# jdm365/Compression_Algorithms

Hardware: AMD Instinct MI355X
Metric: encode GB/s on enwik9 at 1/2/4/8 MI355X; ratio vs ref; round-trip bit-exact (higher is better)
Workload: dtype u8; 1 GPU; deflate (LZ77 W=32 KiB len<=31 + per-block dynamic Huffman over the 286-symbol alphabet, mode H), independent 64 KiB blocks; 1000000000 enwik-shaped bytes in the job, 1000000000 on rank 0; input_seed=12345, mode=H, input_bytes_job=1000000000, input_bytes_rank0=1000000000, compressed_bytes_job=516875560, compressed_bytes_rank0=516875560, gather_to_rank0=False, parallelism=blocks sharded over 1 GPU(s), weak scaling

## Files before the change

compression_algorithms_amd/csrc/lz2.h:

```cpp
#pragma once
#include "lz_common.h"

#define LZ2_NG_BITS   14
#define LZ2_NG        (1u << LZ2_NG_BITS)
#ifndef LZ2_CAP
#define LZ2_CAP       4096u
#endif
#ifndef LZ2_CAP_S
#define LZ2_CAP_S     2048u
#endif
#ifndef LZ2_THREADS
#define LZ2_THREADS   512
#endif
#define LZ2_NWAVES    (LZ2_THREADS / 64)
#ifndef LZ2_PARTBITS
#define LZ2_PARTBITS  7
#endif
#define LZ2_MAXPARTS  (1u << LZ2_PARTBITS)
static_assert(LZ2_CAP % LZ2_THREADS == 0 && LZ2_CAP_S % LZ2_THREADS == 0 && LZ2_CAP_S <= LZ2_CAP, "entries per thread must be whole");
static_assert(2u * (LZ_MAX_BLOCK / LZ2_CAP_S + 1u + 16u) + 2u <= LZ2_MAXPARTS, "a block could need more parts than the partition can number");
#define LZ2_GRID_PARTS 40u
static_assert(LZ2_GRID_PARTS * LZ2_CAP_S >= 5u * LZ_MAX_BLOCK / 4u, "the grid must cover a full block of text with room to spare");
#ifndef LZ2_BIG
#define LZ2_BIG       8u
#endif
#define LZ2_WAVE      128u
#define LZ2_MAXBIG    (LZ2_CAP / LZ2_BIG)
#define LZ2_BIG_STRIDE (2u * LZ_MAX_BLOCK)
#define LZ2_ALIGN8(x)  (((x) + 7u) & ~7u)
#define LZ2_DESC_SMALL (LZ_MAX_BLOCK / LZ2_BIG + 32u)
#define LZ2_NCLASS    8u
#define LZ2_BIG_SMALL 1024u
__host__ __device__ __forceinline__ uint32_t lz2_class_of(uint32_t cnt, uint32_t wave_min)
{
    const bool three = (wave_min >> 16) != 0u;
    wave_min &= 0xFFFFu;
    if (cnt >= wave_min) return cnt > LZ2_BIG_SMALL ? 6u : cnt >= 512u ? 4u : (three && cnt < 256u) ? 3u : 5u;
    return cnt < 16 ? 7u : cnt < 32 ? 0u : cnt < 64 ? 1u : cnt < 128 ? 2u : cnt < 256 ? 3u : 4u;
}

struct Lz2BlockMeta {
    uint32_t n, nparts, base, fallback;
    uint32_t nbig, nbig_entries;
    uint32_t pad[2];
    uint32_t part_start[LZ2_MAXPARTS];
    uint32_t part_count[LZ2_MAXPARTS];
    uint32_t part_lo[LZ2_MAXPARTS];
};

struct Lz2BigDesc {
    uint32_t block;
    uint32_t start;
    uint32_t count;
    uint32_t anom;
    uint32_t limit;
    uint32_t pad[3];
};

struct Lz2Scratch {
    uint8_t      *partmap;
    uint16_t     *plist;
    uint16_t     *cand;
    Lz2BlockMeta *meta;
    uint32_t     *fallback_count, *fallback_list;
    uint32_t     *work_count;
    uint32_t      work_slots;
    uint64_t     *work;
    uint16_t     *bigpos, *bigrs, *bigpid, *bigcand;
    Lz2BigDesc   *desc[LZ2_NCLASS];
    uint32_t     *big_count;
    uint4        *lane_list;
    uint32_t     *lane_hist;
    uint64_t     *dbg;
    uint32_t      wave_min;
    uint32_t      stop_phase;
};
```

compression_algorithms_amd/csrc/lz2_find.hip:

```cpp
#include "lz_common.h"
#include "lz2.h"
#include "lz_dom.h"
#include "lz_replay.h"
#include "internal.h"
#include <stdlib.h>

#define RS_HEAD 0x8000u
#define RS_MASK 0x7FFFu

__device__ __forceinline__ bool bm2_test(const uint32_t *bm, uint32_t b) { return (bm[b >> 5] >> (b & 31u)) & 1u; }

__device__ void replay_small(const uint16_t *pos, uint16_t *rs, const uint16_t *pid, uint16_t *occ, uint32_t *bm,
                             uint32_t s, uint32_t e, uint32_t W, uint32_t anom, uint32_t limit, uint16_t *cand_i)
{
    uint32_t ev = s;
    bool anom_pending = anom != ~0u;
    const bool plain = (anom == ~0u) && (limit == ~0u);
    if (plain && (uint32_t)pos[e - 1] <= (uint32_t)pos[s] + W) {
        for (uint32_t i = s; i < e; ++i) { const uint32_t id = pid[i]; cand_i[i] = (id != pos[i]) ? (uint16_t)id : (uint16_t)LZ_NONE16; }
        return;
    }
    for (uint32_t i = s; i < e; ++i) {
        const uint32_t p = pos[i], rsv = rs[i], r = rsv & RS_MASK, id = pid[i];
        while (ev < i && (uint32_t)pos[ev] + W < p) {
// ... 546 lines not shown
        uint16_t *bp = sc.bigpos + (size_t)lb * LZ2_BIG_STRIDE + dst;
        uint16_t *br = sc.bigrs + (size_t)lb * LZ2_BIG_STRIDE + dst;
        uint16_t *bi = sc.bigpid + (size_t)lb * LZ2_BIG_STRIDE + dst;
        for (uint32_t i = s + (tid & 63); i < e; i += 64) {
            cand_i[i] = e_pos[i];
            bp[i - s] = e_pos[i];
            br[i - s] = (uint16_t)((e_rs[i] & RS_MASK) - s);
            bi[i - s] = e_pid[i];
        }
        uint16_t *bc = sc.bigcand + (size_t)lb * LZ2_BIG_STRIDE + dst;
        for (uint32_t k = (e - s) + (tid & 63); k < LZ2_ALIGN8(e - s); k += 64) { bp[k] = 0; bc[k] = 0; }
    }
    uint16_t *cand_j = s_pid;
    __syncthreads();
    for (uint32_t i = tid; i < m; i += LZ2_THREADS) cand_j[s_j1[i]] = cand_i[i];
    __syncthreads();
    uint16_t *cout = sc.cand + (size_t)lb * LZ_MAX_BLOCK + pstart;
    for (uint32_t j = tid; j < m; j += LZ2_THREADS) cout[j] = cand_j[j];
    LZ2_TICK(6);
    if (LZ2_DBG && tid == 0) atomicAdd((unsigned long long *)&LZ2_DBG[15], 1ull);
}


template <bool DESC>
__device__ __forceinline__ void lz2_find_listed(const uint8_t *__restrict__ in, uint64_t n_total, const LzP &P, const Lz2Scratch &sc, uint64_t block0)
{
    const uint32_t listed = *sc.work_count, nwork = listed < gridDim.x ? listed : gridDim.x;
    const uint32_t cpx = (nwork + 7u) >> 3, item_idx = (blockIdx.x & 7u) * cpx + (blockIdx.x >> 3);
    if ((blockIdx.x >> 3) >= cpx || item_idx >= nwork) return;
    lz2_find_part<LZ2_CAP_S, DESC>(in, n_total, P, sc, block0, sc.work[item_idx]);
}
__global__ __launch_bounds__(LZ2_THREADS, 8)
void k_lz2_find(const uint8_t *__restrict__ in, uint64_t n_total, LzP P, Lz2Scratch sc, uint64_t block0)
{
    lz2_find_listed<false>(in, n_total, P, sc, block0);
}
__global__ __launch_bounds__(LZ2_THREADS, 8)
void k_lz2_find_desc(const uint8_t *__restrict__ in, uint64_t n_total, LzP P, Lz2Scratch sc, uint64_t block0)
{
    lz2_find_listed<true>(in, n_total, P, sc, block0);
}

template <bool DESC>
__global__ __launch_bounds__(LZ2_THREADS)
void k_lz2_find_wide(const uint8_t *__restrict__ in, uint64_t n_total, LzP P, Lz2Scratch sc, uint64_t block0, uint32_t covered)
{
    const uint32_t nwide = sc.work_count[1], listed = sc.work_count[0], rest = listed > covered ? listed - covered : 0u;
    for (uint32_t k = blockIdx.x; k < nwide + rest; k += gridDim.x) {
        lz2_find_part<LZ2_CAP, DESC>(in, n_total, P, sc, block0, k < nwide ? sc.work[sc.work_slots - 1u - k] : sc.work[covered + (k - nwide)]);
        __syncthreads();
    }
}

template <int LDS_ENTRIES, int NW>
__global__ __launch_bounds__(64)
void k_lz2_big(LzP P, Lz2Scratch sc, int large)
{
    __shared__ uint32_t s_occ[LDS_ENTRIES];
    __shared__ uint16_t s_slot[LDS_ENTRIES];
    const uint32_t lane = threadIdx.x;
    const uint32_t nhi = large == 1 ? sc.big_count[6] : (large == 2 || large == 4) ? 0u : sc.big_count[4],
                   ncl = nhi + ((large == 0 || large == 2) ? sc.big_count[5] : large == 4 ? sc.big_count[3] : 0u);
    const uint32_t W = 1u << P.wbits;
    for (uint32_t ci = blockIdx.x; ci < ncl; ci += gridDim.x) {
        const Lz2BigDesc *dp = large == 1 ? &sc.desc[6][ci] : large == 4 ? &sc.desc[3][ci] : (ci < nhi ? &sc.desc[4][ci] : &sc.desc[5][ci - nhi]);
        const uint32_t d_block = dp->block, d_start = dp->start, n = dp->count;
        if (n & 0x80000000u) continue;
        const uint32_t d_anom = dp->anom, d_limit = dp->limit;
        const uint16_t *bp = sc.bigpos + (size_t)d_block * LZ2_BIG_STRIDE + d_start;
        const uint16_t *br = sc.bigrs + (size_t)d_block * LZ2_BIG_STRIDE + d_start;
        const uint16_t *bi = sc.bigpid + (size_t)d_block * LZ2_BIG_STRIDE + d_start;
        uint16_t *bc = sc.bigcand + (size_t)d_block * LZ2_BIG_STRIDE + d_start;
        const bool plain = d_anom == ~0u && d_limit == ~0u;
        if constexpr (NW > 1) {
            if (n <= 2048u) {
                if (plain) big_replay<LDS_ENTRIES, 1, true>(s_occ, s_slot, lane, W, n, d_anom, d_limit, bp, br, bi, bc);
                else big_replay<LDS_ENTRIES, 1, false>(s_occ, s_slot, lane, W, n, d_anom, d_limit, bp, br, bi, bc);
                continue;
            }
            if (n <= 4096u) {
                if (plain) big_replay<LDS_ENTRIES, 2, true>(s_occ, s_slot, lane, W, n, d_anom, d_limit, bp, br, bi, bc);
                else big_replay<LDS_ENTRIES, 2, false>(s_occ, s_slot, lane, W, n, d_anom, d_limit, bp, br, bi, bc);
                continue;
            }
        }
        if (plain) big_replay<LDS_ENTRIES, NW, true>(s_occ, s_slot, lane, W, n, d_anom, d_limit, bp, br, bi, bc);
        else big_replay<LDS_ENTRIES, NW, false>(s_occ, s_slot, lane, W, n, d_anom, d_limit, bp, br, bi, bc);
    }
}

#define LZ2_DOM_DONE 0x80000000u
__global__ __launch_bounds__(256)
void k_lz2_dom(LzP P, Lz2Scratch sc)
{
    constexpr uint32_t RING = LZ2_CAP;
    static_assert((RING & (RING - 1u)) == 0, "the ring is indexed with a mask");
    __shared__ uint32_t s_occ[LZ2_CAP / 32 + 72 + 264];
    __shared__ uint16_t s_ring[RING];
    __shared__ uint16_t s_fid[DOM_FCAP], s_fpos[DOM_FCAP], s_fslot[DOM_FCAP];
    __shared__ uint32_t s_votes[3], s_result, s_next;
    const uint32_t tid = threadIdx.x;
    const uint32_t W = 1u << P.wbits;
    const uint32_t count = sc.big_count[6];
    uint32_t *cursor = sc.big_count + 8;
    struct Src {
        const uint16_t *bp, *br, *bi; uint16_t *bc;
        __device__ __forceinline__ uint64_t ent(uint32_t i) const { return ((uint64_t)bp[i] << 16) | ((uint64_t)br[i] << 32) | ((uint64_t)bi[i] << 48); }
        __device__ __forceinline__ void put(uint32_t i, uint32_t, uint32_t res) const { bc[i] = (uint16_t)res; }
    };
    for (;;) {
        __syncthreads();
        if (tid == 0) s_next = atomicAdd(cursor, 1u);
        __syncthreads();
        const uint32_t ci = s_next;
        if (ci >= count) break;
        Lz2BigDesc *dp = &sc.desc[6][ci];
        const uint32_t m = dp->count;
        if (dp->anom != ~0u || dp->limit != ~0u || m > LZ2_CAP) continue;
        const size_t at = (size_t)dp->block * LZ2_BIG_STRIDE + dp->start;
        Src src{sc.bigpos + at, sc.bigrs + at, sc.bigpid + at, sc.bigcand + at};
        for (uint32_t i = tid; i < m; i += 256) src.bc[i] = (uint16_t)LZ_NONE16;
        if (tid == 0) { s_votes[0] = s_votes[1] = s_votes[2] = 0; s_result = 0; }
        __syncthreads();
        const bool done = dom_cluster(src, m, W, (W < RING ? W : RING) - 1u, s_occ, s_ring, s_fid, s_fpos, s_fslot, s_votes, s_result, nullptr);
        if (done && tid == 0) dp->count = m | LZ2_DOM_DONE;
    }
}

#define ROW_BPERM(src_lane, v) ((uint32_t)__builtin_amdgcn_ds_bpermute((int)((src_lane) << 2), (int)(v)))

template <int RL>
__device__ __forceinline__ uint32_t row_first_zero(uint32_t v, uint32_t from, uint32_t l, uint32_t rb)
{
    constexpr uint32_t RMASK = RL == 32 ? 0xFFFFFFFFu : ((1u << (RL & 31)) - 1u);
    const uint32_t rw = from >> 5, lowmask = (1u << (from & 31u)) - 1u;
    if (l < rw) v = 0xFFFFFFFFu; else if (l == rw) v |= lowmask;
    const uint64_t mk = __ballot(v != 0xFFFFFFFFu);
    const uint32_t my = (uint32_t)(mk >> rb) & RMASK;
    const uint32_t ln = my ? (uint32_t)__builtin_ctz(my) : 0u;
    const uint32_t mv = ROW_BPERM(rb + ln, v);
    const uint32_t fz = (mv != 0xFFFFFFFFu) ? (uint32_t)__builtin_ctz(~mv) : 0u;
    return my ? ((ln << 5) + fz) : ~0u;
}

template <int RL>
__global__ __launch_bounds__(64)
void k_lz2_rows(LzP P, Lz2Scratch sc, int cls_a, int cls_b, int cursor_slot)
{
    static_assert(RL == 8 || RL == 16 || RL == 32, "rows of 8, 16 or 32 lanes");
    constexpr int NR = 64 / RL, CAPE = 32 * RL;
    constexpr uint32_t RMASK = RL == 32 ? 0xFFFFFFFFu : ((1u << (RL & 31)) - 1u);
    __shared__ uint32_t s_occ[NR][CAPE];
    __shared__ uint32_t s_ent[NR][CAPE];
    __shared__ uint32_t s_bm[NR][RL];
    const uint32_t lane = threadIdx.x, g = lane / (uint32_t)RL, l = lane & (uint32_t)(RL - 1), rb = lane & ~(uint32_t)(RL - 1);
    const uint32_t W = 1u << P.wbits;
    const uint32_t count_a = sc.big_count[cls_a], count = count_a + sc.big_count[cls_b];
    uint32_t *cursor = sc.big_count + cursor_slot;
    Lz2BigDesc *const descs_a = sc.desc[cls_a], *const descs_b = sc.desc[cls_b];
    auto desc_of = [&](uint32_t ticket) -> Lz2BigDesc * { return ticket < count_a ? descs_a + ticket : descs_b + (ticket - count_a); };
    uint32_t *occ = s_occ[g], *ent = s_ent[g], *bmw = s_bm[g];

    bool active = false, exhausted = false;
    uint32_t n = 0, i0 = 0, ev = 0;
    size_t at = 0;
    uint32_t cur_a = 0, cur_b = 0, out_acc = LZ_NONE16;
    uint32_t pf_stage = 0, pf_ci = 0, pf_count = 0;
    size_t pf_at = 0;
    uint32_t r_np = 0, r_ni = 0, r_nr = 0, r_fp = 0, r_fi = 0, r_fr = 0, tk = 0;
    uint4 r_d4 = make_uint4(0, 0, 0, 0); uint32_t r_d1 = 0;
    uint32_t vzero;
    asm volatile("v_mov_b32 %0, 0" : "=v"(vzero));

    for (;;) {
        const bool flush = active && i0 + l < n;
        uint16_t *const flush_to = sc.bigcand + at + i0 + l;
        if (active) {
            i0 += (uint32_t)RL;
            if (i0 >= n) active = false;
            else { cur_a = r_np | (r_ni << 16); cur_b = r_nr; }
        }
        bool take = false, want_cursor = false;
        uint32_t done_ci = 0, done_n = 0;
        if (!active && pf_stage == 3u) {
            take = true;
            n = pf_count; at = pf_at;
            cur_a = r_fp | (r_fi << 16); cur_b = r_fr; i0 = 0; ev = 0; active = true; pf_stage = 0;
            bmw[l] = 0;
            done_ci = pf_ci; done_n = n;
        }
        if (pf_stage == 1u) {
            pf_ci = ROW_BPERM(rb, tk);
            if (pf_ci >= count) { exhausted = true; pf_stage = 0; } else pf_stage = 2;
        } else if (pf_stage == 2u) {
            if (r_d4.w != ~0u || r_d1 != ~0u || r_d4.z > (uint32_t)CAPE || r_d4.z < 2u * RL) pf_stage = 0;
            else { pf_count = r_d4.z; pf_at = (size_t)r_d4.x * LZ2_BIG_STRIDE + r_d4.y; pf_stage = 3; }
        }
        if (pf_stage == 0u && !exhausted) { want_cursor = true; pf_stage = 1; }
        {
            const uint32_t k = i0 + (uint32_t)RL + l;
            const size_t na = (active && k < n) ? at + k : 0;
            r_np = sc.bigpos[na]; r_ni = sc.bigpid[na]; r_nr = sc.bigrs[na];
            const size_t fa = (pf_stage == 3u) ? pf_at + l : 0;
            r_fp = sc.bigpos[fa]; r_fi = sc.bigpid[fa]; r_fr = sc.bigrs[fa];
            const uint32_t *dp = reinterpret_cast<const uint32_t *>(pf_stage == 2u ? desc_of(pf_ci) : descs_a);
            r_d4 = *reinterpret_cast<const uint4 *>(dp); r_d1 = dp[4];
        }
        if (flush) *flush_to = (uint16_t)out_acc;
        if (take && l == 0) desc_of(done_ci)->count = done_n | LZ2_DOM_DONE;
        if (want_cursor && l == 0) tk = atomicAdd(cursor + vzero, 1u);
        if (__ballot(active || pf_stage != 0u) == 0ull) break;
        if (__ballot(active) == 0ull) continue;
        uint32_t a = ROW_BPERM(rb, cur_a), r = ROW_BPERM(rb, cur_b);
        uint32_t e = ent[(active && ev + l < i0) ? ev + l : 0u];
        for (uint32_t t = 0; t < (uint32_t)RL; ++t) {
            const uint32_t i = i0 + t;
            const bool on = active && i < n;
            const uint32_t p = a & 0xFFFFu, id = a >> 16;
            for (;;) {
                const bool ret = on && ev + l < i && (e >> 16) + W < p;
                const uint64_t mk = __ballot(ret);
                if (ret) atomicAnd(&bmw[(e & 0xFFFFu) >> 5], ~(1u << (e & 31u)));
                const uint32_t cnt = (uint32_t)__popc((uint32_t)(mk >> rb) & RMASK);
                ev += cnt;
                if (__ballot(cnt == (uint32_t)RL) == 0ull) break;
                e = ent[(on && ev + l < i) ? ev + l : 0u];
            }
            const uint32_t wr = bmw[r >> 5], h = occ[r], v = bmw[l];
            const uint32_t tn = (t + 1u) & (uint32_t)(RL - 1);
            const uint32_t na = ROW_BPERM(rb + tn, cur_a), nr = ROW_BPERM(rb + tn, cur_b);
            const bool bit = (wr >> (r & 31u)) & 1u, same = (h & 0xFFFFu) == id;
            const bool seek = on && id != p;
            uint32_t res = (seek && ev == 0u) ? id : (seek && bit && same) ? (h >> 16) : (uint32_t)LZ_NONE16;
            bool walk = seek && ev != 0u && bit && !same;
            if (__ballot(walk) != 0ull) {
                uint32_t e_end = row_first_zero<RL>(v, r + 1u, l, rb);
                if (e_end > (uint32_t)CAPE) e_end = (uint32_t)CAPE;
                uint32_t b0 = r + 1u;
                while (__ballot(walk && b0 < e_end) != 0ull) {
                    const uint32_t bb = b0 + l;
                    const bool in = walk && bb < e_end;
                    const uint32_t o = occ[in ? bb : 0u];
                    const uint64_t mk = __ballot(in && (o & 0xFFFFu) == id);
                    const uint32_t my = (uint32_t)(mk >> rb) & RMASK;
                    const uint32_t src = ROW_BPERM(rb + (my ? (uint32_t)__builtin_ctz(my) : 0u), o);
                    if (walk && my) { res = src >> 16; walk = false; }
                    b0 += (uint32_t)RL;
                }
            }
            const uint32_t b = row_first_zero<RL>(v, r, l, rb);
            const bool put = on && b < (uint32_t)CAPE;
            if (put && l == 0) atomicOr(&bmw[b >> 5], 1u << (b & 31u));
            if (put) { occ[b] = id | (p << 16); ent[i] = b | (p << 16); }
            if (on && l == t) out_acc = res;
            e = ent[(active && i + 1u < n && ev + l < i + 1u) ? ev + l : 0u];
            a = na; r = nr;
            __builtin_amdgcn_wave_barrier();
        }
    }
}

__device__ __forceinline__ uint32_t u16_of(const uint4 &v, uint32_t k)
{
    const uint64_t lo = (uint64_t)v.x | ((uint64_t)v.y << 32), hi = (uint64_t)v.z | ((uint64_t)v.w << 32);
    return (uint32_t)(((k & 4u) ? hi : lo) >> ((k & 3u) * 16u)) & 0xFFFFu;
}

constexpr uint32_t LANE_SIZES = LZ2_WAVE;

__host__ __device__ __forceinline__ uint32_t lz2_lane_region(uint32_t n)
// ... 147 lines not shown
    }
}

__global__ __launch_bounds__(1024)
void k_lz2_scatter(Lz2Scratch sc, uint16_t *__restrict__ cand_by_pos )
{
    const uint32_t lb = blockIdx.x;
    const Lz2BlockMeta *mt = sc.meta + lb;
    if (mt->fallback) return;
    const uint32_t n = mt->n;
    const uint16_t *pl = sc.plist + (size_t)lb * LZ_MAX_BLOCK, *cd = sc.cand + (size_t)lb * LZ_MAX_BLOCK;
    uint16_t *out = cand_by_pos + (size_t)lb * LZ_MAX_BLOCK;
    for (uint32_t j = threadIdx.x; j < n; j += 1024) { const uint32_t c = cd[j], p = pl[j]; if (c != p || p == LZ_NONE16) out[p] = (uint16_t)c; }
    __syncthreads();
    const uint32_t nb = mt->nbig_entries;
    const uint16_t *bp = sc.bigpos + (size_t)lb * LZ2_BIG_STRIDE, *bc = sc.bigcand + (size_t)lb * LZ2_BIG_STRIDE;
    for (uint32_t j = threadIdx.x; j < nb; j += 1024) { const uint32_t p = bp[j], c = bc[j]; if (c != p) out[p] = (uint16_t)c; }
}

template __global__ void k_lz2_big<LZ2_BIG_SMALL, 1>(LzP, Lz2Scratch, int);
template __global__ void k_lz2_big<512, 1>(LzP, Lz2Scratch, int);
template __global__ void k_lz2_big<256, 1>(LzP, Lz2Scratch, int);
template __global__ void k_lz2_big<LZ2_CAP, 4>(LzP, Lz2Scratch, int);
template __global__ void k_lz2_rows<16>(LzP, Lz2Scratch, int, int, int);


static uint32_t lz2_class_cap(uint32_t c)
{
    static const uint32_t lo[LZ2_NCLASS] = {16, 32, 64, 128, 256, 128, 1025, 8};
    return LZ_MAX_BLOCK / lo[c] + 8;
}

void lz2_carve(mi_carver &cv, uint32_t nb, Lz2Scratch *sc)
{
    sc->partmap = cv.take<uint8_t>((size_t)nb * LZ_MAX_BLOCK);
    sc->plist = cv.take<uint16_t>((size_t)nb * LZ_MAX_BLOCK);
    sc->cand = cv.take<uint16_t>((size_t)nb * LZ_MAX_BLOCK);
    sc->meta = cv.take<Lz2BlockMeta>(nb);
    sc->fallback_count = cv.take<uint32_t>(64 + 2 * LANE_SIZES);
    sc->fallback_list = cv.take<uint32_t>(nb);
    sc->bigpos = cv.take<uint16_t>((size_t)nb * LZ2_BIG_STRIDE);
    sc->bigrs = cv.take<uint16_t>((size_t)nb * LZ2_BIG_STRIDE);
    sc->bigpid = cv.take<uint16_t>((size_t)nb * LZ2_BIG_STRIDE);
    sc->bigcand = cv.take<uint16_t>((size_t)nb * LZ2_BIG_STRIDE);
    for (uint32_t c = 0; c < LZ2_NCLASS; ++c) sc->desc[c] = cv.take<Lz2BigDesc>((size_t)nb * lz2_class_cap(c));
    sc->big_count = cv.at(sc->fallback_count, 16);
    sc->work_count = cv.at(sc->fallback_count, 32);
    sc->lane_hist = cv.at(sc->fallback_count, 64);
    sc->work = cv.take<uint64_t>((size_t)nb * LZ2_MAXPARTS);
    sc->work_slots = nb * LZ2_MAXPARTS;
    sc->lane_list = cv.take<uint4>((size_t)nb * lz2_class_cap(7));
    sc->dbg = getenv("MI_LZ_DEBUG") ? cv.take<uint64_t>(64) : nullptr;
    { const char *e = getenv("MI_LZ_ROWS"); const uint32_t rows = e ? (uint32_t)atoi(e) : 1u; sc->wave_min = LZ2_WAVE | ((rows ? 1u : 0u) << 16); }
#ifdef MI_MEASURE
    sc->stop_phase = getenv("MI_LZ_STOP_PHASE") ? (uint32_t)atoi(getenv("MI_LZ_STOP_PHASE")) : 0u;
#else
    sc->stop_phase = 0u;
#endif
}

static uint32_t lz2_env_u32(const char *name, uint32_t dflt)
{
    const char *e = getenv(name);
    if (!e) return dflt;
    const long v = atol(e);
    return v >= 0 ? (uint32_t)v : dflt;
}

extern "C" int mi_lz_debug_counters(mi_ctx *ctx, uint64_t *out32)
{
    if (!ctx || !ctx->lz_dbg) return 0;
    (void)hipDeviceSynchronize();
    return hipMemcpy(out32, ctx->lz_dbg, 64 * 8, hipMemcpyDeviceToHost) == hipSuccess ? 1 : 0;
}

mi_status lz2_stage_partition(mi_ctx *ctx, const LzP &P, const uint8_t *d_in, uint64_t n, uint64_t block0, uint32_t nb,
                              const Lz2Scratch &sc, hipStream_t s)
{
    MI_HIP(ctx, hipMemsetAsync(sc.fallback_count, 0, (64 + 2 * LANE_SIZES) * 4, s));
    if (sc.dbg && ctx->lz_dbg != sc.dbg) { ctx->lz_dbg = sc.dbg; MI_HIP(ctx, hipMemsetAsync(sc.dbg, 0, 512, s)); }
    mi_prof_scope p(ctx, "k_lz2_partition", s, (uint64_t)nb * P.block);
    lz2_launch_partition(d_in, n, P, sc, block0, nb, s);
    MI_HIP(ctx, hipGetLastError());
    return MI_OK;
}

static uint32_t lz2_find_grid(const LzP &P, uint32_t nb)
{
    const uint32_t parts = P.block / 64u + 1u < LZ2_GRID_PARTS ? P.block / 64u + 1u : LZ2_GRID_PARTS;
    return (parts * nb + 7u) & ~7u;
}

mi_status lz2_stage_find(mi_ctx *ctx, const LzP &P, const uint8_t *d_in, uint64_t n, uint64_t block0, uint32_t nb,
                         const Lz2Scratch &sc, hipStream_t s)
{
    mi_prof_scope p(ctx, "k_lz2_find", s, (uint64_t)nb * P.block);
    if (P.flags & LZP_DESC) hipLaunchKernelGGL(k_lz2_find_desc, dim3(lz2_find_grid(P, nb)), dim3(LZ2_THREADS), 0, s, d_in, n, P, sc, block0);
    else hipLaunchKernelGGL(k_lz2_find, dim3(lz2_find_grid(P, nb)), dim3(LZ2_THREADS), 0, s, d_in, n, P, sc, block0);
    MI_HIP(ctx, hipGetLastError());
    return MI_OK;
}

mi_status lz2_stage_find_wide(mi_ctx *ctx, const LzP &P, const uint8_t *d_in, uint64_t n, uint64_t block0, uint32_t nb,
                              const Lz2Scratch &sc, hipStream_t s, bool aside)
{
    static const bool prof_fb = getenv("MI_LZ_PROF_FALLBACK") != nullptr;
    const int saved_prof = ctx->profiling;
    if (aside && !prof_fb) ctx->profiling = 0;
    {
        mi_prof_scope p(ctx, "k_lz2_find_wide", s, (uint64_t)nb * P.block);
        if (P.flags & LZP_DESC) hipLaunchKernelGGL(k_lz2_find_wide<true>, dim3(256), dim3(LZ2_THREADS), 0, s, d_in, n, P, sc, block0, lz2_find_grid(P, nb));
        else hipLaunchKernelGGL(k_lz2_find_wide<false>, dim3(256), dim3(LZ2_THREADS), 0, s, d_in, n, P, sc, block0, lz2_find_grid(P, nb));
    }
    ctx->profiling = saved_prof;
    MI_HIP(ctx, hipGetLastError());
    return MI_OK;
}

mi_status lz2_stage_b(mi_ctx *ctx, const LzP &P, uint32_t nb, const Lz2Scratch &sc, hipStream_t s, int which)
{
    const uint32_t ncu = (uint32_t)ctx->num_cu;
    auto grid_of = [](uint64_t worst) -> uint32_t { return (uint32_t)(worst ? worst : 1); };
    if (which & 4) {
        static const uint32_t kib_env = lz2_env_u32("MI_LZ_LANES_KIB", 8);
        const uint32_t kib = kib_env < 1u ? 1u : kib_env > 32u ? 32u : kib_env, budget_dw = kib * 256u;
        const uint64_t worst = (uint64_t)nb * lz2_class_cap(7);
        const uint32_t og = (uint32_t)((worst + 255u) / 256u < (uint64_t)ncu * 4u ? (worst + 255u) / 256u : (uint64_t)ncu * 4u);
        { mi_prof_scope p(ctx, "k_lz2_lane_order", s, (uint64_t)nb * P.block);
          hipLaunchKernelGGL(k_lz2_lane_count, dim3(og), dim3(256), 0, s, sc);
          hipLaunchKernelGGL(k_lz2_lane_place, dim3(og), dim3(256), 0, s, P, sc); }
        uint32_t m = ~0u;
        for (uint32_t c = LZ2_BIG; c < LANE_SIZES; ++c) { const uint32_t x = c * lz2_lane_width(c, budget_dw); m = x < m ? x : m; }
        const uint64_t waves = (uint64_t)nb * LZ_MAX_BLOCK / m + LANE_SIZES;
        { mi_prof_scope p(ctx, "k_lz2_lanes", s, (uint64_t)nb * P.block);
          hipLaunchKernelGGL(k_lz2_lanes, dim3((uint32_t)waves), dim3(64), budget_dw * 4u, s, P, sc, LANE_SIZES - 1u, LZ2_BIG, budget_dw); }
    }
    if (which & 2) {
    { mi_prof_scope p(ctx, "k_lz2_big", s, (uint64_t)nb * P.block);
      static const bool split = !(getenv("MI_LZ_BIG_SPLIT") && getenv("MI_LZ_BIG_SPLIT")[0] == '0');
      const uint32_t rows = sc.wave_min >> 16;
      static const uint32_t rows_waves = lz2_env_u32("MI_LZ_ROWS_WAVES", 9);
      if (rows >= 1 && split && (sc.wave_min & 0xFFFFu) == LZ2_WAVE) {
          hipLaunchKernelGGL((k_lz2_big<LZ2_BIG_SMALL, 1>), dim3(grid_of((uint64_t)nb * lz2_class_cap(4))), dim3(64), 0, s, P, sc, 3);
          hipLaunchKernelGGL((k_lz2_rows<16>), dim3(ncu * rows_waves), dim3(64), 0, s, P, sc, 5, 3, 9);
          hipLaunchKernelGGL((k_lz2_big<512, 1>), dim3(ncu * 4u), dim3(64), 0, s, P, sc, 2);
          hipLaunchKernelGGL((k_lz2_big<256, 1>), dim3(ncu * 4u), dim3(64), 0, s, P, sc, 4);
      } else if (split && (sc.wave_min & 0xFFFFu) == LZ2_WAVE) {
          hipLaunchKernelGGL((k_lz2_big<LZ2_BIG_SMALL, 1>), dim3(grid_of((uint64_t)nb * lz2_class_cap(4))), dim3(64), 0, s, P, sc, 3);
          hipLaunchKernelGGL((k_lz2_big<512, 1>), dim3(grid_of((uint64_t)nb * lz2_class_cap(5))), dim3(64), 0, s, P, sc, 2);
      } else {
          hipLaunchKernelGGL((k_lz2_big<LZ2_BIG_SMALL, 1>), dim3(grid_of((uint64_t)nb * (lz2_class_cap(4) + lz2_class_cap(5)))), dim3(64), 0, s, P, sc, 0);
          if (rows) hipLaunchKernelGGL((k_lz2_big<256, 1>), dim3(grid_of((uint64_t)nb * lz2_class_cap(3))), dim3(64), 0, s, P, sc, 4);
      } }
    { mi_prof_scope p(ctx, "k_lz2_dom", s, (uint64_t)nb * P.block);
      const uint64_t worst = (uint64_t)nb * lz2_class_cap(6);
      hipLaunchKernelGGL(k_lz2_dom, dim3((unsigned)(worst < (uint64_t)ncu * 4u ? worst : (uint64_t)ncu * 4u)), dim3(256), 0, s, P, sc); }
    { mi_prof_scope p(ctx, "k_lz2_big<4096>", s, (uint64_t)nb * P.block);
      hipLaunchKernelGGL((k_lz2_big<LZ2_CAP, 4>), dim3(grid_of((uint64_t)nb * lz2_class_cap(6) < 4096 ? (uint64_t)nb * lz2_class_cap(6) : 4096)), dim3(64), 0, s, P, sc, 1); }
    }
    MI_HIP(ctx, hipGetLastError());
    return MI_OK;
}

void lz2_launch_scatter(const Lz2Scratch &sc, uint16_t *cand_by_pos, uint32_t nb, hipStream_t s)
{
    hipLaunchKernelGGL(k_lz2_scatter, dim3(nb), dim3(1024), 0, s, sc, cand_by_pos);
}
```

compression_algorithms_amd/csrc/lz_replay.h:

```cpp
#pragma once
#include "lz_common.h"

#define RLANE(v, l) ((uint32_t)__builtin_amdgcn_readlane((int)(v), (int)(l)))

#define WB_SWITCH(q, OP) switch (q) { case 0: OP(0); break; case 1: OP(1); break; case 2: OP(2); break; case 3: OP(3); break; case 4: OP(4); break; case 5: OP(5); break; case 6: OP(6); break; case 7: OP(7); break; case 8: OP(8); break; case 9: OP(9); break; case 10: OP(10); break; case 11: OP(11); break; case 12: OP(12); break; case 13: OP(13); break; case 14: OP(14); break; case 15: OP(15); break; case 16: OP(16); break; case 17: OP(17); break; case 18: OP(18); break; case 19: OP(19); break; case 20: OP(20); break; case 21: OP(21); break; case 22: OP(22); break; case 23: OP(23); break; case 24: OP(24); break; case 25: OP(25); break; case 26: OP(26); break; case 27: OP(27); break; case 28: OP(28); break; case 29: OP(29); break; case 30: OP(30); break; case 31: OP(31); break; default: break; }

template <int NW>
struct WaveBitmap {
    uint32_t w[NW];
    uint32_t full;
    __device__ __forceinline__ void clear() {
#pragma unroll
        for (int q = 0; q < NW; ++q) w[q] = 0;
        full = 0;
    }
    template <int K> __device__ __forceinline__ uint32_t reg_lane(uint32_t ln) const { if constexpr (K < NW) return RLANE(w[K], ln); else return 0u; }
    template <int K> __device__ __forceinline__ void reg_and(uint32_t keep) { if constexpr (K < NW) w[K] &= keep; }
    template <int K> __device__ __forceinline__ void reg_set(uint32_t bit) {
        if constexpr (K < NW) { w[K] |= bit; if (__ballot(w[K] != 0xFFFFFFFFu) == 0ull) full |= 1u << K; }
    }
    template <int K> __device__ __forceinline__ uint32_t reg_first_zero(uint32_t rw, uint32_t lowmask, uint32_t lane) const {
        if constexpr (K < NW) {
            const uint32_t wi = (uint32_t)K * 64u + lane;
            uint32_t v = w[K];
// ... 29 lines not shown
            full &= ~(1u << wq);
        } else {
#pragma unroll
            for (int q = 0; q < NW; ++q) w[q] &= (NW == 1 || (uint32_t)q == wq) ? keep : 0xFFFFFFFFu;
        }
    }
    __device__ __forceinline__ void flip(uint32_t slot, uint32_t lane) {
        const uint32_t wi = slot >> 5, wq = wi >> 6;
        const uint32_t bit = (lane == (wi & 63u)) ? (1u << (slot & 31u)) : 0u;
        if constexpr (NW > 4) {
#define OP(K) reg_set<K>(bit)
            WB_SWITCH(wq, OP)
#undef OP
        } else {
#pragma unroll
            for (int q = 0; q < NW; ++q) w[q] ^= (NW == 1 || (uint32_t)q == wq) ? bit : 0u;
        }
    }
    __device__ __forceinline__ uint32_t first_zero_from(uint32_t r, uint32_t lane) const {
        const uint32_t rw = r >> 5, lowmask = (1u << (r & 31u)) - 1u;
        uint32_t res = ~0u;
        if constexpr (NW > 4) {
            uint32_t q = rw >> 6;
            while (q < (uint32_t)NW) {
#define OP(K) res = reg_first_zero<K>(rw, lowmask, lane)
                WB_SWITCH(q, OP)
#undef OP
                if (res != ~0u) break;
                const uint32_t rest = (q + 1u < 32u) ? (~full >> (q + 1u)) : 0u;
                if (!rest) break;
                q = q + 1u + (uint32_t)__builtin_ctz(rest);
            }
            return res;
        }
        bool found = false;
#pragma unroll
        for (int q = 0; q < NW; ++q) {
            const uint32_t wi = (uint32_t)q * 64u + lane;
            uint32_t v = w[q];
            if (wi < rw) v = 0xFFFFFFFFu; else if (wi == rw) v |= lowmask;
            const uint64_t nz = __ballot(v != 0xFFFFFFFFu);
            if (!found && nz) {
                const uint32_t ln = (uint32_t)__builtin_ctzll(nz);
                const uint32_t mv = RLANE(v, ln);
                res = (((uint32_t)q * 64u + ln) << 5) + (uint32_t)__builtin_ctz(~mv);
                found = true;
            }
        }
        return res;
    }
};


template <int LDS_ENTRIES, int NW, bool PLAIN>
__device__ __forceinline__ void big_replay(uint32_t *s_occ, uint16_t *s_slot, uint32_t lane, uint32_t W, uint32_t n,
                                           uint32_t d_anom, uint32_t d_limit, const uint16_t *bp, const uint16_t *br,
                                           const uint16_t *bi, uint16_t *bc)
{
    WaveBitmap<NW> bm;
    bm.clear();
    uint32_t ev = 0;
    bool anom_pending = !PLAIN && d_anom != ~0u;
    uint32_t c_pos = 0, c_rs = 0, c_pid = 0, out_acc = 0;
    uint32_t ev_pos = lane < n ? bp[lane] : 0u;
    uint32_t pe = RLANE(ev_pos, 0);
    uint32_t n_pos = ev_pos, n_rs = 0, n_pid = 0;
    if (lane < n) { n_rs = br[lane]; n_pid = bi[lane]; }
    for (uint32_t i0 = 0; i0 < n; i0 += 64) {
        const uint32_t ii = i0 + lane;
        c_pos = n_pos; c_rs = n_rs; c_pid = n_pid;
        if (ii + 64 < n) { n_pos = bp[ii + 64]; n_rs = br[ii + 64]; n_pid = bi[ii + 64]; }
        const uint32_t lim = (n - i0) < 64u ? (n - i0) : 64u;
        for (uint32_t t = 0; t < lim; ++t) {
            const uint32_t i = i0 + t;
            const uint32_t p = RLANE(c_pos, t), r = RLANE(c_rs, t), id = RLANE(c_pid, t);
            while (ev < i && pe + W < p) {
                const uint32_t sl = (uint32_t)__builtin_amdgcn_readfirstlane((int)s_slot[ev]);
                bm.clear_bit(sl, lane);
                ++ev;
                if ((ev & 63u) == 0) { const uint32_t q = ev + lane; ev_pos = q < n ? bp[q] : 0u; }
                pe = RLANE(ev_pos, ev & 63u);
            }
            if (!PLAIN && anom_pending && p > W - 1u) { bm.clear_bit(d_anom, lane); anom_pending = false; }
            uint32_t res = LZ_NONE16;
            if (PLAIN && ev == 0) {
                if (id != p) res = id;
            } else if (id != p) {
                const uint32_t h = (uint32_t)__builtin_amdgcn_readfirstlane((int)s_occ[r]);
                if (bm.test(r)) {
                    if ((h & 0xFFFFu) == id) res = h >> 16;
                    else {
                        uint32_t e = bm.first_zero_from(r + 1u, lane);
                        if (e > (uint32_t)LDS_ENTRIES) e = (uint32_t)LDS_ENTRIES;
                        if (!PLAIN && r < d_limit && d_limit < e) e = d_limit;
                        for (uint32_t b0 = r + 1u; b0 < e; b0 += 64u) {
                            const uint32_t b = b0 + lane;
                            const uint32_t o = b < e ? s_occ[b] : 0u;
                            const uint64_t hit = __ballot(b < e && (o & 0xFFFFu) == id);
                            if (hit) { res = RLANE(o, (uint32_t)__builtin_ctzll(hit)) >> 16; break; }
                        }
                    }
                }
            }
            const uint32_t b = bm.first_zero_from(r, lane);
            bm.flip(b, lane);
            s_occ[b] = id | (p << 16); s_slot[i] = (uint16_t)b;
            if (lane == t) out_acc = res;
            __builtin_amdgcn_wave_barrier();
        }
        if (ii < n) bc[ii] = (uint16_t)out_acc;
    }
    __builtin_amdgcn_wave_barrier();
}


template <bool PLAIN>
__device__ __forceinline__ void huge_replay(uint16_t *s_oid, uint32_t lane, uint32_t W, uint32_t n, uint32_t d_anom, uint32_t d_limit,
                                            const uint16_t *bp, const uint16_t *br, const uint16_t *bi, uint16_t *bc,
                                            uint16_t *gslot, uint16_t *gopos)
{
    constexpr uint32_t CAPS = 65536u;
    WaveBitmap<32> bm;
    bm.clear();
    uint32_t ev = 0;
    bool anom_pending = !PLAIN && d_anom != ~0u;
    uint32_t c_pos = 0, c_rs = 0, c_pid = 0, out_acc = 0;
    uint32_t ev_pos = lane < n ? bp[lane] : 0u;
    uint32_t pe = RLANE(ev_pos, 0);
    uint32_t ev_slot = 0, ev_slot_base = ~0u, ev_slot_upto = 0;
    uint32_t an_slot = ~0u, an_pos = 0, cb_slot = ~0u, cb_pos = 0;
    uint32_t n_pos = ev_pos, n_rs = 0, n_pid = 0;
    if (lane < n) { n_rs = br[lane]; n_pid = bi[lane]; }
    for (uint32_t i0 = 0; i0 < n; i0 += 64) {
        const uint32_t ii = i0 + lane;
        c_pos = n_pos; c_rs = n_rs; c_pid = n_pid;
        if (ii + 64 < n) { n_pos = bp[ii + 64]; n_rs = br[ii + 64]; n_pid = bi[ii + 64]; }
        const uint32_t lim = (n - i0) < 64u ? (n - i0) : 64u;
        for (uint32_t t = 0; t < lim; ++t) {
            const uint32_t i = i0 + t;
            const uint32_t p = RLANE(c_pos, t), r = RLANE(c_rs, t), id = RLANE(c_pid, t);
            while (ev < i && pe + W < p) {
                if ((ev & ~63u) != ev_slot_base || ev >= ev_slot_upto) {
                    __threadfence();
                    ev_slot_base = ev & ~63u;
                    const uint32_t q = ev_slot_base + lane;
                    ev_slot = q < i ? (uint32_t)__builtin_nontemporal_load(gslot + q) : 0u;
                    ev_slot_upto = i;
                }
                const uint32_t sl = RLANE(ev_slot, ev & 63u);
                bm.clear_bit(sl, lane);
                ++ev;
                if ((ev & 63u) == 0) { const uint32_t q = ev + lane; ev_pos = q < n ? bp[q] : 0u; }
                pe = RLANE(ev_pos, ev & 63u);
            }
            if (!PLAIN && anom_pending && p > W - 1u) { bm.clear_bit(d_anom, lane); anom_pending = false; }
            uint32_t res = LZ_NONE16;
            if (PLAIN && ev == 0) {
                if (id != p) res = id;
            } else if (id != p) {
                const uint32_t h = (uint32_t)__builtin_amdgcn_readfirstlane((int)s_oid[r]);
                if (bm.test(r)) {
                    uint32_t hit = ~0u;
                    if (h == id) hit = r;
// ... 38 lines not shown
```

Measured before the change: 24.58 GB/s.

## Precompute eviction-free replay prefix in parallel before big and dom replay

Adds a k_lz2_prefix kernel that, for plain clusters of up to 1024 entries, handles the leading stretch of entries whose positions all lie within one window of the first. In that stretch no eviction happens, so candidates equal the pid and slots can be assigned in parallel with ballots instead of one entry at a time. The kernel writes the candidates and slots, records the prefix length in the descriptor, and marks fully covered clusters done. The big and dom replay kernels then rebuild their occupancy state from the stored slots and continue serially from the prefix. This adds a kernel launch and extra state-reload traffic in exchange for less serial per-entry replay work.

```diff
diff --git a/compression_algorithms_amd/csrc/lz2.h b/compression_algorithms_amd/csrc/lz2.h
--- a/compression_algorithms_amd/csrc/lz2.h
+++ b/compression_algorithms_amd/csrc/lz2.h
@@ -74,4 +74,5 @@
     uint64_t     *dbg;
     uint32_t      wave_min;
     uint32_t      stop_phase;
+    uint32_t      prefix;
 };
diff --git a/compression_algorithms_amd/csrc/lz2_find.hip b/compression_algorithms_amd/csrc/lz2_find.hip
--- a/compression_algorithms_amd/csrc/lz2_find.hip
+++ b/compression_algorithms_amd/csrc/lz2_find.hip
@@ -622,6 +622,77 @@
     }
 }
 
+#define LZ2_DOM_DONE 0x80000000u
+#ifdef MI_TEST_HOOKS
+__device__ unsigned long long g_lz2_prefix_stats[2];
+#define LZ2_PREFIX_COUNT(who, entries) do { if (who) { atomicAdd(&g_lz2_prefix_stats[0], 1ull); atomicAdd(&g_lz2_prefix_stats[1], (unsigned long long)(entries)); } } while (0)
+#else
+#define LZ2_PREFIX_COUNT(who, entries) do { } while (0)
+#endif
+
+__global__ __launch_bounds__(64)
+void k_lz2_prefix(LzP P, Lz2Scratch sc)
+{
+    const uint32_t lane = threadIdx.x;
+    const uint32_t W = 1u << P.wbits;
+    const uint32_t n4 = sc.big_count[4], n5 = sc.big_count[5], ncl = n4 + n5 + sc.big_count[3];
+    auto desc_of = [&](uint32_t c) -> Lz2BigDesc * { return c < n4 ? sc.desc[4] + c : c < n4 + n5 ? sc.desc[5] + (c - n4) : sc.desc[3] + (c - n4 - n5); };
+    auto ours = [](const uint4 &d, uint32_t limit) -> bool { return d.z != 0u && d.z <= LZ2_BIG_SMALL && d.w == ~0u && limit == ~0u; };
+    for (uint32_t ci = blockIdx.x; ci < ncl; ci += gridDim.x) {
+        Lz2BigDesc *dp = desc_of(ci);
+        const uint4 c_a = *reinterpret_cast<const uint4 *>(dp);
+        if (!ours(c_a, dp->limit)) continue;
+        const uint32_t n = (uint32_t)__builtin_amdgcn_readfirstlane((int)c_a.z);
+        const size_t at = (size_t)c_a.x * LZ2_BIG_STRIDE + c_a.y;
+        const uint16_t *bp = sc.bigpos + at, *bi = sc.bigpid + at;
+        uint16_t *br = sc.bigrs + at, *bc = sc.bigcand + at;
+        uint32_t bm = 0;
+        uint32_t pre = 0;
+        uint32_t n_pos = 0, n_rs = 0, n_pid = 0;
+        if (lane < n) { n_pos = bp[lane]; n_rs = br[lane]; n_pid = bi[lane]; }
+        const uint32_t last = RLANE(n_pos, 0) + W;
+        for (uint32_t i0 = 0; i0 < n; i0 += 64) {
+            const uint32_t ii = i0 + lane;
+            const uint32_t c_pos = n_pos, c_rs = n_rs, c_pid = n_pid;
+            if (ii + 64 < n) { n_pos = bp[ii + 64]; n_rs = br[ii + 64]; n_pid = bi[ii + 64]; }
+            const uint64_t inside = __ballot(ii < n && c_pos <= last);
+            const uint32_t lim = ~inside ? (uint32_t)__builtin_ctzll(~inside) : 64u;
+            if (lim == 0u) break;
+            if (lane < lim) bc[ii] = (uint16_t)(c_pid == c_pos ? (uint32_t)LZ_NONE16 : c_pid);
+            const uint32_t below = (uint32_t)__shfl_up((int)c_rs, 1);
+            const uint64_t heads = __ballot(lane < lim && (lane == 0u || c_rs != below));
+            bool stuck = false;
+            for (uint32_t t = 0; t < lim;) {
+                const uint32_t r = RLANE(c_rs, t);
+                const uint64_t rest = t + 1u < 64u ? heads >> (t + 1u) : 0ull;
+                const uint32_t run = rest ? (uint32_t)__builtin_ctzll(rest) + 1u : lim - t;
+                const uint32_t rw = r >> 5;
+                uint32_t v = bm;
+                if (lane < rw) v = 0xFFFFFFFFu; else if (lane == rw) v |= (1u << (r & 31u)) - 1u;
+                const uint64_t nz = __ballot(v != 0xFFFFFFFFu);
+                if (!nz) { stuck = true; break; }
+                const uint32_t wl = (uint32_t)__builtin_ctzll(nz);
+                const uint32_t f = ~RLANE(v, wl);
+                const uint32_t fc = (uint32_t)__popc(f), m = run < fc ? run : fc;
+                const uint32_t rank = (uint32_t)__popc(f & ((1u << (lane & 31u)) - 1u));
+                const bool mine = lane < 32u && ((f >> (lane & 31u)) & 1u) && rank < m;
+                const uint32_t taken = (uint32_t)__ballot(mine);
+                if (mine) br[i0 + t + rank] = (uint16_t)((wl << 5) + lane);
+                if (lane == wl) bm |= taken;
+                t += m;
+            }
+            if (stuck) { lz_order_violation(P); break; }
+            pre += lim;
+            if (lim < 64u) break;
+        }
+        if (lane == 0) {
+            dp->pad[1] = pre;
+            if (pre == n) dp->count = n | LZ2_DOM_DONE;
+        }
+        LZ2_PREFIX_COUNT(lane == 0 && pre == n, pre);
+    }
+}
+
 template <int LDS_ENTRIES, int NW>
 __global__ __launch_bounds__(64)
 void k_lz2_big(LzP P, Lz2Scratch sc, int large)
@@ -642,6 +713,15 @@
         const uint16_t *bi = sc.bigpid + (size_t)d_block * LZ2_BIG_STRIDE + d_start;
         uint16_t *bc = sc.bigcand + (size_t)d_block * LZ2_BIG_STRIDE + d_start;
         const bool plain = d_anom == ~0u && d_limit == ~0u;
+        if constexpr (NW == 1) {
+            __shared__ uint32_t s_stage[64];
+            const uint32_t pre = dp->pad[1];
+            if (plain && pre != 0u && pre < n) {
+                LZ2_PREFIX_COUNT(lane == 0, pre);
+                big_replay<LDS_ENTRIES, 1, true, true>(s_occ, s_slot, lane, W, n, d_anom, d_limit, bp, br, bi, bc, pre, s_stage);
+                continue;
+            }
+        }
         if constexpr (NW > 1) {
             if (n <= 2048u) {
                 if (plain) big_replay<LDS_ENTRIES, 1, true>(s_occ, s_slot, lane, W, n, d_anom, d_limit, bp, br, bi, bc);
@@ -659,7 +739,6 @@
     }
 }
 
-#define LZ2_DOM_DONE 0x80000000u
 __global__ __launch_bounds__(256)
 void k_lz2_dom(LzP P, Lz2Scratch sc)
 {
@@ -732,18 +811,18 @@
     uint32_t *occ = s_occ[g], *ent = s_ent[g], *bmw = s_bm[g];
 
     bool active = false, exhausted = false;
-    uint32_t n = 0, i0 = 0, ev = 0;
+    uint32_t n = 0, i0 = 0, ev = 0, pre = 0;
     size_t at = 0;
     uint32_t cur_a = 0, cur_b = 0, out_acc = LZ_NONE16;
-    uint32_t pf_stage = 0, pf_ci = 0, pf_count = 0;
+    uint32_t pf_stage = 0, pf_ci = 0, pf_count = 0, pf_pre = 0;
     size_t pf_at = 0;
     uint32_t r_np = 0, r_ni = 0, r_nr = 0, r_fp = 0, r_fi = 0, r_fr = 0, tk = 0;
-    uint4 r_d4 = make_uint4(0, 0, 0, 0); uint32_t r_d1 = 0;
+    uint4 r_d4 = make_uint4(0, 0, 0, 0); uint32_t r_d1 = 0, r_d6 = 0;
     uint32_t vzero;
     asm volatile("v_mov_b32 %0, 0" : "=v"(vzero));
 
     for (;;) {
-        const bool flush = active && i0 + l < n;
+        const bool flush = active && i0 + l < n && i0 + l >= pre;
         uint16_t *const flush_to = sc.bigcand + at + i0 + l;
         if (active) {
             i0 += (uint32_t)RL;
@@ -754,8 +833,8 @@
         uint32_t done_ci = 0, done_n = 0;
         if (!active && pf_stage == 3u) {
             take = true;
-            n = pf_count; at = pf_at;
-            cur_a = r_fp | (r_fi << 16); cur_b = r_fr; i0 = 0; ev = 0; active = true; pf_stage = 0;
+            n = pf_count; at = pf_at; pre = pf_pre;
+            cur_a = r_fp | (r_fi << 16); cur_b = r_fr; i0 = pre & ~(uint32_t)(RL - 1); ev = 0; active = true; pf_stage = 0;
             bmw[l] = 0;
             done_ci = pf_ci; done_n = n;
         }
@@ -764,28 +843,57 @@
             if (pf_ci >= count) { exhausted = true; pf_stage = 0; } else pf_stage = 2;
         } else if (pf_stage == 2u) {
             if (r_d4.w != ~0u || r_d1 != ~0u || r_d4.z > (uint32_t)CAPE || r_d4.z < 2u * RL) pf_stage = 0;
-            else { pf_count = r_d4.z; pf_at = (size_t)r_d4.x * LZ2_BIG_STRIDE + r_d4.y; pf_stage = 3; }
+            else { pf_count = r_d4.z; pf_at = (size_t)r_d4.x * LZ2_BIG_STRIDE + r_d4.y; pf_pre = r_d6 < r_d4.z ? r_d6 : 0u; pf_stage = 3; }
         }
         if (pf_stage == 0u && !exhausted) { want_cursor = true; pf_stage = 1; }
         {
             const uint32_t k = i0 + (uint32_t)RL + l;
             const size_t na = (active && k < n) ? at + k : 0;
             r_np = sc.bigpos[na]; r_ni = sc.bigpid[na]; r_nr = sc.bigrs[na];
-            const size_t fa = (pf_stage == 3u) ? pf_at + l : 0;
+            const uint32_t fk = (pf_pre & ~(uint32_t)(RL - 1)) + l;
+            const size_t fa = (pf_stage == 3u && fk < pf_count) ? pf_at + fk : 0;
             r_fp = sc.bigpos[fa]; r_fi = sc.bigpid[fa]; r_fr = sc.bigrs[fa];
             const uint32_t *dp = reinterpret_cast<const uint32_t *>(pf_stage == 2u ? desc_of(pf_ci) : descs_a);
-            r_d4 = *reinterpret_cast<const uint4 *>(dp); r_d1 = dp[4];
+            r_d4 = *reinterpret_cast<const uint4 *>(dp); r_d1 = dp[4]; r_d6 = dp[6];
         }
         if (flush) *flush_to = (uint16_t)out_acc;
         if (take && l == 0) desc_of(done_ci)->count = done_n | LZ2_DOM_DONE;
         if (want_cursor && l == 0) tk = atomicAdd(cursor + vzero, 1u);
+        {
+            uint64_t starts = __ballot(take && l == 0 && pre != 0u);
+            while (starts) {
+                const uint32_t src = (uint32_t)__builtin_ctzll(starts), g2 = src / (uint32_t)RL;
+                starts &= starts - 1ull;
+                const uint32_t pre2 = RLANE(pre, src);
+                const size_t at2 = (size_t)RLANE((uint32_t)at, src) | ((size_t)RLANE((uint32_t)((uint64_t)at >> 32), src) << 32);
+                LZ2_PREFIX_COUNT(lane == 0, pre2);
+                for (uint32_t j0 = 0; j0 < pre2; j0 += 256u) {
+                    uint32_t sl[4], pp[4], idw[4];
+#pragma unroll
+                    for (uint32_t u = 0; u < 4u; ++u) {
+                        const uint32_t j = j0 + 64u * u + lane;
+                        const size_t ja = j < pre2 ? at2 + j : 0;
+                        sl[u] = sc.bigrs[ja]; pp[u] = sc.bigpos[ja]; idw[u] = sc.bigpid[ja];
+                    }
+#pragma unroll
+                    for (uint32_t u = 0; u < 4u; ++u) {
+                        const uint32_t j = j0 + 64u * u + lane;
+                        if (j < pre2 && sl[u] < (uint32_t)CAPE) {
+                            s_occ[g2][sl[u]] = idw[u] | (pp[u] << 16); s_ent[g2][j] = sl[u] | (pp[u] << 16);
+                            atomicOr(&s_bm[g2][sl[u] >> 5], 1u << (sl[u] & 31u));
+                        }
+                    }
+                }
+            }
+            __builtin_amdgcn_wave_barrier();
+        }
         if (__ballot(active || pf_stage != 0u) == 0ull) break;
         if (__ballot(active) == 0ull) continue;
         uint32_t a = ROW_BPERM(rb, cur_a), r = ROW_BPERM(rb, cur_b);
         uint32_t e = ent[(active && ev + l < i0) ? ev + l : 0u];
         for (uint32_t t = 0; t < (uint32_t)RL; ++t) {
             const uint32_t i = i0 + t;
-            const bool on = active && i < n;
+            const bool on = active && i < n && i >= pre;
             const uint32_t p = a & 0xFFFFu, id = a >> 16;
             for (;;) {
                 const bool ret = on && ev + l < i && (e >> 16) + W < p;
@@ -1039,6 +1147,7 @@
     sc->lane_list = cv.take<uint4>((size_t)nb * lz2_class_cap(7));
     sc->dbg = getenv("MI_LZ_DEBUG") ? cv.take<uint64_t>(64) : nullptr;
     { const char *e = getenv("MI_LZ_ROWS"); const uint32_t rows = e ? (uint32_t)atoi(e) : 1u; sc->wave_min = LZ2_WAVE | ((rows ? 1u : 0u) << 16); }
+    { const char *e = getenv("MI_LZ_PREFIX"); sc->prefix = e ? (atoi(e) ? 1u : 0u) : 1u; }
 #ifdef MI_MEASURE
     sc->stop_phase = getenv("MI_LZ_STOP_PHASE") ? (uint32_t)atoi(getenv("MI_LZ_STOP_PHASE")) : 0u;
 #else
@@ -1060,6 +1169,19 @@
     (void)hipDeviceSynchronize();
     return hipMemcpy(out32, ctx->lz_dbg, 64 * 8, hipMemcpyDeviceToHost) == hipSuccess ? 1 : 0;
 }
+
+#ifdef MI_TEST_HOOKS
+extern "C" int mi_test_prefix_stats(mi_ctx *ctx, uint64_t *out2, int reset)
+{
+    if (!ctx || !out2) return 0;
+    unsigned long long h[2] = {0, 0};
+    if (hipDeviceSynchronize() != hipSuccess) return 0;
+    if (hipMemcpyFromSymbol(h, HIP_SYMBOL(g_lz2_prefix_stats), sizeof h) != hipSuccess) return 0;
+    out2[0] = h[0]; out2[1] = h[1];
+    if (reset) { h[0] = h[1] = 0; if (hipMemcpyToSymbol(HIP_SYMBOL(g_lz2_prefix_stats), h, sizeof h) != hipSuccess) return 0; }
+    return 1;
+}
+#endif
 
 mi_status lz2_stage_partition(mi_ctx *ctx, const LzP &P, const uint8_t *d_in, uint64_t n, uint64_t block0, uint32_t nb,
                               const Lz2Scratch &sc, hipStream_t s)
@@ -1123,6 +1245,9 @@
           hipLaunchKernelGGL(k_lz2_lanes, dim3((uint32_t)waves), dim3(64), budget_dw * 4u, s, P, sc, LANE_SIZES - 1u, LZ2_BIG, budget_dw); }
     }
     if (which & 2) {
+    if (sc.prefix) { mi_prof_scope p(ctx, "k_lz2_prefix", s, (uint64_t)nb * P.block);
+      const uint64_t worst = (uint64_t)nb * (lz2_class_cap(3) + lz2_class_cap(4) + lz2_class_cap(5));
+      hipLaunchKernelGGL(k_lz2_prefix, dim3((unsigned)(worst < (uint64_t)ncu * 32u ? worst : (uint64_t)ncu * 32u)), dim3(64), 0, s, P, sc); }
     { mi_prof_scope p(ctx, "k_lz2_big", s, (uint64_t)nb * P.block);
       static const bool split = !(getenv("MI_LZ_BIG_SPLIT") && getenv("MI_LZ_BIG_SPLIT")[0] == '0');
       const uint32_t rows = sc.wave_min >> 16;
diff --git a/compression_algorithms_amd/csrc/lz_replay.h b/compression_algorithms_amd/csrc/lz_replay.h
--- a/compression_algorithms_amd/csrc/lz_replay.h
+++ b/compression_algorithms_amd/csrc/lz_replay.h
@@ -105,11 +105,12 @@
 };
 
 
-template <int LDS_ENTRIES, int NW, bool PLAIN>
+template <int LDS_ENTRIES, int NW, bool PLAIN, bool PRE = false>
 __device__ __forceinline__ void big_replay(uint32_t *s_occ, uint16_t *s_slot, uint32_t lane, uint32_t W, uint32_t n,
                                            uint32_t d_anom, uint32_t d_limit, const uint16_t *bp, const uint16_t *br,
-                                           const uint16_t *bi, uint16_t *bc)
+                                           const uint16_t *bi, uint16_t *bc, uint32_t pre = 0, uint32_t *s_stage = nullptr)
 {
+    static_assert(!PRE || (PLAIN && NW == 1), "a precomputed prefix: plain clusters of the one-register classes only");
     WaveBitmap<NW> bm;
     bm.clear();
     uint32_t ev = 0;
@@ -118,13 +119,37 @@
     uint32_t ev_pos = lane < n ? bp[lane] : 0u;
     uint32_t pe = RLANE(ev_pos, 0);
     uint32_t n_pos = ev_pos, n_rs = 0, n_pid = 0;
-    if (lane < n) { n_rs = br[lane]; n_pid = bi[lane]; }
-    for (uint32_t i0 = 0; i0 < n; i0 += 64) {
+    uint32_t i_first = 0;
+    if constexpr (PRE) {
+        i_first = pre & ~63u;
+        const uint32_t q = i_first + lane;
+        n_pos = 0;
+        if (q < n) { n_pos = bp[q]; n_rs = br[q]; n_pid = bi[q]; }
+        s_stage[lane] = 0;
+        for (uint32_t j0 = 0; j0 < pre; j0 += 256) {
+            uint32_t sl[4] = {0, 0, 0, 0}, pp[4] = {0, 0, 0, 0}, idw[4] = {0, 0, 0, 0};
+#pragma unroll
+            for (uint32_t u = 0; u < 4u; ++u) { const uint32_t j = j0 + 64u * u + lane; if (j < pre) { sl[u] = br[j]; pp[u] = bp[j]; idw[u] = bi[j]; } }
+#pragma unroll
+            for (uint32_t u = 0; u < 4u; ++u) {
+                const uint32_t j = j0 + 64u * u + lane;
+                if (j < pre) {
+                    if (sl[u] < (uint32_t)LDS_ENTRIES) { s_occ[sl[u]] = idw[u] | (pp[u] << 16); atomicOr(&s_stage[sl[u] >> 5], 1u << (sl[u] & 31u)); }
+                    s_slot[j] = (uint16_t)sl[u];
+                }
+            }
+        }
+        __builtin_amdgcn_wave_barrier();
+        bm.w[0] = s_stage[lane];
+    } else if (lane < n) { n_rs = br[lane]; n_pid = bi[lane]; }
+    for (uint32_t i0 = i_first; i0 < n; i0 += 64) {
         const uint32_t ii = i0 + lane;
         c_pos = n_pos; c_rs = n_rs; c_pid = n_pid;
         if (ii + 64 < n) { n_pos = bp[ii + 64]; n_rs = br[ii + 64]; n_pid = bi[ii + 64]; }
         const uint32_t lim = (n - i0) < 64u ? (n - i0) : 64u;
-        for (uint32_t t = 0; t < lim; ++t) {
+        uint32_t t_first = 0;
+        if constexpr (PRE) t_first = pre > i0 ? pre - i0 : 0u;
+        for (uint32_t t = t_first; t < lim; ++t) {
             const uint32_t i = i0 + t;
             const uint32_t p = RLANE(c_pos, t), r = RLANE(c_rs, t), id = RLANE(c_pid, t);
             while (ev < i && pe + W < p) {
@@ -136,7 +161,7 @@
             }
             if (!PLAIN && anom_pending && p > W - 1u) { bm.clear_bit(d_anom, lane); anom_pending = false; }
             uint32_t res = LZ_NONE16;
-            if (PLAIN && ev == 0) {
+            if (!PRE && PLAIN && ev == 0) {
                 if (id != p) res = id;
             } else if (id != p) {
                 const uint32_t h = (uint32_t)__builtin_amdgcn_readfirstlane((int)s_occ[r]);
@@ -161,7 +186,7 @@
             if (lane == t) out_acc = res;
             __builtin_amdgcn_wave_barrier();
         }
-        if (ii < n) bc[ii] = (uint16_t)out_acc;
+        if (ii < n && (!PRE || ii >= pre)) bc[ii] = (uint16_t)out_acc;
     }
     __builtin_amdgcn_wave_barrier();
 }
```

Result: faster. 24.99 GB/s, median of 6 (+1.7%).
